# teofum/rust_raytracer

Hardware: AMD Instinct MI355X
Metric: Msamples/sec (whole node), cornell_dragon 870k tri @1000spp (higher is better)
Workload: dtype f64; 1 GPU; scenes/cornell_dragon 1200x1200 @1000spp (10 replicas x 10x10 strata), 871200-tri stand-in mesh; spp=1000, seed=1, pipeline=auto, frames_in_flight=1, partition=1200-row bands round-robin over 1 GPU(s)

## Files before the change

include/rt_mi355.h:

```cpp
#ifndef RT_MI355_H
#define RT_MI355_H

#include <stdint.h>
#include <stddef.h>

#ifdef __cplusplus
extern "C" {
#endif

#define RT_MI355_ABI_VERSION 2

typedef enum RtStatus {
    RT_OK = 0,
    RT_E_INVALID = -1,
    RT_E_UNSUPPORTED = -2,
    RT_E_DEVICE = -3,
    RT_E_NOMEM = -4
} RtStatus;

typedef enum RtNodeType {
    RT_NODE_SPHERE = 1,
    RT_NODE_PLANE = 2,
    RT_NODE_MESH = 3,
    RT_NODE_LIST = 4,
// ... 175 lines not shown
                     const RtRenderParams* params, double* d_rgba_out, void* stream);

int rt_get_stats(const RtScene* scene, RtRenderStats* out);

int rt_debug_trace_sample(const RtScene* scene, const RtCameraDesc* camera, const RtRenderParams* params,
                          uint32_t tid, uint32_t x, uint32_t y, uint32_t sx, uint32_t sy,
                          double* rgb_out, double* trace_out, uint32_t max_bounces);

int rt_debug_fuzzy_reflection(int device, uint32_t n, const double* reflected, const double* fuzz, const uint64_t* state, double* out, uint64_t* state_out);

#define RT_SCENE_INFO_ZERO_WEIGHT_STOP 1u
#define RT_SCENE_INFO_TEX_INTERPRETER 2u
#define RT_SCENE_INFO_VOLUMES 4u
int rt_scene_info(const RtSceneDesc* desc, uint32_t* flags_out);
int rt_scene_mesh_stats(const RtSceneDesc* desc, uint64_t out[8]);
int rt_scene_program(const RtSceneDesc* desc, int32_t* ops_out, uint32_t capacity, uint32_t* n_ops_out, uint64_t info[8]);

int rt_scene_set_tail_flag(RtScene* scene, int32_t* flag);

typedef struct RtAccum RtAccum;
int rt_accum_create(const RtScene* scene, const RtCameraDesc* camera, const RtRenderParams* params, RtAccum** out);
void rt_accum_destroy(RtAccum* acc);
int rt_accum_render(RtAccum* acc, uint32_t n_replicas, const RtRenderParams* params_or_null, void* stream);
uint32_t rt_accum_replicas_done(const RtAccum* acc);
int rt_accum_estimate(const RtAccum* acc, double* rgba_out);
int rt_accum_estimate_device(const RtAccum* acc, double* d_rgba_out, void* stream);
int rt_accum_preview_rgb8(const RtAccum* acc, uint8_t* rgb_out);
size_t rt_accum_state_size(const RtAccum* acc);
int rt_accum_save_state(const RtAccum* acc, void* buf, size_t size);
int rt_accum_load_state(RtAccum* acc, const void* buf, size_t size);
// ... 48 lines not shown
```

rust_raytracer_amd/api.py:

```python
from __future__ import annotations

import ctypes as C
import os
import sys
from typing import Optional, Sequence

import numpy as np

PKG_DIR = os.path.dirname(os.path.abspath(__file__))
REPO_DIR = os.path.dirname(PKG_DIR)

RT_OK = 0
RT_E_INVALID, RT_E_UNSUPPORTED, RT_E_DEVICE, RT_E_NOMEM = -1, -2, -3, -4
RT_PRECISION_F64, RT_PRECISION_F32 = 0, 1
RT_PIPELINE_AUTO, RT_PIPELINE_MEGAKERNEL, RT_PIPELINE_WAVEFRONT = 0, 1, 2
RT_SCENE_BVH_ON_DEVICE = 1
RT_DENOISE_DEMODULATE = 1
RT_DENOISE_MAX_ITERATIONS = 16
AOV_CHANNELS = 8

(RT_NODE_SPHERE, RT_NODE_PLANE, RT_NODE_MESH, RT_NODE_LIST, RT_NODE_TRANSFORM, RT_NODE_BVH,
 RT_NODE_SKY, RT_NODE_SUN, RT_NODE_VOLUME, RT_NODE_NULL) = range(1, 11)
(RT_MAT_LAMBERTIAN, RT_MAT_METAL, RT_MAT_DIELECTRIC, RT_MAT_GLOSSY, RT_MAT_EMISSIVE,
 RT_MAT_ISOTROPIC, RT_MAT_NORMAL_DEBUG) = range(1, 8)
(RT_TEX_CONST_COLOR, RT_TEX_CONST_FLOAT, RT_TEX_CHECKER, RT_TEX_CHECKER_SOLID, RT_TEX_LERP,
 RT_TEX_IMAGE, RT_TEX_NOISE_SOLID, RT_TEX_CHANNEL, RT_TEX_UV_DEBUG) = range(1, 10)


class RtNode(C.Structure):
    _fields_ = [("type", C.c_uint32), ("flags", C.c_uint32), ("material", C.c_int32),
                ("mesh", C.c_int32), ("transform", C.c_int32), ("first_child", C.c_uint32),
# ... 196 lines not shown
        lib.rt_render_device.restype = C.c_int
        lib.rt_get_stats.argtypes = [C.c_void_p, C.POINTER(RtRenderStats)]
        lib.rt_get_stats.restype = C.c_int
        lib.rt_debug_trace_sample.argtypes = [C.c_void_p, C.POINTER(RtCameraDesc), C.POINTER(RtRenderParams),
                                              C.c_uint32, C.c_uint32, C.c_uint32, C.c_uint32, C.c_uint32,
                                              C.POINTER(C.c_double), C.POINTER(C.c_double), C.c_uint32]
        lib.rt_debug_trace_sample.restype = C.c_int
        lib.rt_scene_info.argtypes = [C.POINTER(RtSceneDesc), C.POINTER(C.c_uint32)]
        lib.rt_scene_info.restype = C.c_int
        if hasattr(lib, "rt_scene_set_tail_flag"):
            lib.rt_scene_set_tail_flag.argtypes = [C.c_void_p, C.c_void_p]
            lib.rt_scene_set_tail_flag.restype = C.c_int
        if hasattr(lib, "rt_scene_mesh_stats"):
            lib.rt_scene_mesh_stats.argtypes = [C.POINTER(RtSceneDesc), C.POINTER(C.c_uint64)]
            lib.rt_scene_mesh_stats.restype = C.c_int
        if hasattr(lib, "rt_accum_create"):
            for name, res, args in (
                    ("rt_accum_create", C.c_int, [C.c_void_p, C.POINTER(RtCameraDesc), C.POINTER(RtRenderParams), C.POINTER(C.c_void_p)]),
                    ("rt_accum_destroy", None, [C.c_void_p]),
                    ("rt_accum_render", C.c_int, [C.c_void_p, C.c_uint32, C.POINTER(RtRenderParams), C.c_void_p]),
                    ("rt_accum_replicas_done", C.c_uint32, [C.c_void_p]),
                    ("rt_accum_estimate", C.c_int, [C.c_void_p, C.c_void_p]),
                    ("rt_accum_estimate_device", C.c_int, [C.c_void_p, C.c_void_p, C.c_void_p]),
                    ("rt_accum_preview_rgb8", C.c_int, [C.c_void_p, C.c_void_p]),
                    ("rt_accum_state_size", C.c_size_t, [C.c_void_p]),
                    ("rt_accum_save_state", C.c_int, [C.c_void_p, C.c_void_p, C.c_size_t]),
                    ("rt_accum_load_state", C.c_int, [C.c_void_p, C.c_void_p, C.c_size_t]),
                    ("rt_tonemap_rgb8_device", C.c_int, [C.c_int, C.c_void_p, C.c_uint32, C.c_uint32, C.c_void_p, C.c_void_p])):
                fn = getattr(lib, name)
                fn.argtypes = args
# ... 39 lines not shown
    if st != RT_OK:
        raise RtError(st, lib.rt_last_error().decode())
    return flags.value


def scene_mesh_stats(desc) -> dict:
    lib = load_device_lib()
    out = (C.c_uint64 * 8)()
    st = lib.rt_scene_mesh_stats(desc, out)
    if st != RT_OK:
        raise RtError(st, lib.rt_last_error().decode())
    return dict(zip(("triangles", "bvh2_nodes", "bvh4_nodes", "bvh2_depth", "bvh4_stack", "ops", "rebuilt_groups", "rebuilt_prims"),
                    [int(x) for x in out]))


def scene_program(desc) -> tuple:
    import numpy as np
    lib = load_device_lib()
    lib.rt_scene_program.argtypes = [C.POINTER(RtSceneDesc), C.POINTER(C.c_int32), C.c_uint32, C.POINTER(C.c_uint32), C.POINTER(C.c_uint64)]
    lib.rt_scene_program.restype = C.c_int
    n = C.c_uint32()
    info = (C.c_uint64 * 8)()
    st = lib.rt_scene_program(desc, None, 0, C.byref(n), info)
    if st != RT_OK:
        raise RtError(st, lib.rt_last_error().decode())
    ops = np.zeros((n.value, 4), dtype=np.int32)
    st = lib.rt_scene_program(desc, ops.ctypes.data_as(C.POINTER(C.c_int32)), n.value, C.byref(n), info)
    if st != RT_OK:
        raise RtError(st, lib.rt_last_error().decode())
    plan = int(info[6])
# ... 360 lines not shown
```

rust_raytracer_amd/csrc/rt_bvh.cpp:

```cpp
#include "rt_bvh.h"

#include <algorithm>
#include <cmath>
#include <cstdlib>
#include <limits>

#include "rt_scene.h"

namespace rt {
namespace {

constexpr int kMaxBins = 64;
static int g_bins = 16;
constexpr double kInf = std::numeric_limits<double>::infinity();

struct Box {
    double lo[3] = {kInf, kInf, kInf};
    double hi[3] = {-kInf, -kInf, -kInf};
    void grow(const double* p) {
        for (int a = 0; a < 3; a++) {
            if (p[a] < lo[a]) lo[a] = p[a];
            if (p[a] > hi[a]) hi[a] = p[a];
        }
    }
// ... 214 lines not shown
    c.build(0, 0, 0);
    for (int a = 0; a < 3; a++) { c.out.root_lo[a] = kInf; c.out.root_hi[a] = -kInf; }
    const BuildNodeN<W>& r = c.out.nodes[0];
    for (int k = 0; k < W; k++)
        if (r.child[k] != kEmptyChild)
            for (int a = 0; a < 3; a++) {
                c.out.root_lo[a] = std::min(c.out.root_lo[a], r.lo[k][a]);
                c.out.root_hi[a] = std::max(c.out.root_hi[a], r.hi[k][a]);
            }
    return std::move(c.out);
}
}

Bvh4Build collapse_bvh4(const BvhBuild& b2) { return collapse<4>(b2); }

}
```

rust_raytracer_amd/csrc/rt_bvh.h:

```cpp
#pragma once
#include <cstdint>
#include <string>
#include <vector>

namespace rt {

struct BuildNode {
    double lo0[3], hi0[3], lo1[3], hi1[3];
    int32_t c0, c1;
};

struct BvhBuild {
    std::vector<BuildNode> nodes;
    std::vector<uint32_t> tri_order;
    uint32_t max_depth = 0;
};

BvhBuild build_bvh(const double* positions, const uint32_t* tri_pos, uint32_t n_tris, uint32_t max_leaf);

bool build_bvh_device(const double* positions, uint32_t n_positions, const uint32_t* tri_pos, uint32_t n_tris, uint32_t max_leaf,
                      BvhBuild* out, std::string* err);

template <int W>
struct BuildNodeN {
    double lo[W][3], hi[W][3];
    int32_t child[W];
};
template <int W>
struct BvhNBuild {
    std::vector<BuildNodeN<W>> nodes;
    uint32_t max_depth = 0;
    uint32_t max_stack = 0;
    double root_lo[3], root_hi[3];
};
using BuildNode4 = BuildNodeN<4>;
using Bvh4Build = BvhNBuild<4>;
Bvh4Build collapse_bvh4(const BvhBuild& bvh2);

}
```

rust_raytracer_amd/csrc/rt_kernels.hip:

```cpp
#include <hip/hip_runtime.h>

#include <algorithm>
#include <cmath>
#include <cstdio>
#include <cstdlib>
#include <cstring>
#include <memory>
#include <new>
#include <string>
#include <type_traits>
#include <vector>

#include "rt_aov.h"
#include "rt_compile.h"
#include "rt_device.h"
#include "rt_wavefront.h"

namespace rt {

template <typename R, bool STATS, bool TEX>
__global__ void __launch_bounds__(256) k_megakernel(SceneView<R> sc, CameraView<R> cam, ParamsView<R> prm,
                                                    double* __restrict__ out, DeviceCounters* counters, uint32_t t_first,
                                                    uint32_t n_rep) {
    extern __shared__ int lds_stack[];
// ... 327 lines not shown
            group_nodes.resize(cs.group_nodes4.size());
            for (size_t g = 0; g < cs.groups.size(); g++) {
                const GroupRec<double>& gr = cs.groups[g];
                double S = 0.0;
                for (int a = 0; a < 3; a++) S = std::fmax(S, std::fmax(std::fabs(gr.lo[a]), std::fabs(gr.hi[a])));
                if (!std::isfinite(S)) return set_err(RT_E_UNSUPPORTED, "primitive group with an unbounded box");
                const size_t end = g + 1 < cs.groups.size() ? cs.groups[g + 1].root : cs.group_nodes4.size();
                for (size_t i = gr.root; i < end; i++) {
                    const BuildNode4& sn = cs.group_nodes4[i];
                    BvhNode4q& qn = group_nodes[i];
                    if (!quantise(4, sn.lo, sn.hi, sn.child, S * (1.0 / 524288.0), qn.org, qn.cell, qn.qlo, qn.qhi, qn.child))
                        return set_err(RT_E_UNSUPPORTED, "group BVH node does not fit the 8-bit grid");
                }
            }
        }
        std::vector<Bounds<R>> mesh_bounds(cs.mesh_bounds.size());
        for (size_t i = 0; i < mesh_bounds.size(); i++)
            for (int a = 0; a < 3; a++) {
                mesh_bounds[i].lo[a] = round_down<R>(cs.mesh_bounds[i].lo[a]);
                mesh_bounds[i].hi[a] = round_up<R>(cs.mesh_bounds[i].hi[a]);
            }
        std::vector<TriRec<R>> tris(cs.tris.size());
        for (size_t i = 0; i < tris.size(); i++) {
            cast_arr(tris[i].v0, cs.tris[i].v0); cast_arr(tris[i].e1, cs.tris[i].e1); cast_arr(tris[i].e2, cs.tris[i].e2);
            tris[i]._pad = R(0);
        }
        std::vector<TriAttr<R>> attrs(cs.attrs.size());
        for (size_t i = 0; i < attrs.size(); i++) {
            const auto& s = cs.attrs[i];
            cast_arr(attrs[i].n0, s.n0); cast_arr(attrs[i].n1, s.n1); cast_arr(attrs[i].n2, s.n2);
// ... 28 lines not shown
        std::vector<R> perlin_vec(cs.perlin_vec.size());
        for (size_t i = 0; i < perlin_vec.size(); i++) perlin_vec[i] = R(cs.perlin_vec[i]);
        int st;
        if ((st = buf.upload(cs.ops, &view.ops)) != RT_OK) return st;
        if ((st = buf.upload(bounds, &view.bounds)) != RT_OK) return st;
        if ((st = buf.upload(cs.chain_offsets, &view.chain_offsets)) != RT_OK) return st;
        if ((st = buf.upload(cs.chain_items, &view.chain_items)) != RT_OK) return st;
        if ((st = buf.upload(xforms, &view.xforms)) != RT_OK) return st;
        if ((st = buf.upload(spheres, &view.spheres)) != RT_OK) return st;
        if ((st = buf.upload(planes, &view.planes)) != RT_OK) return st;
        if ((st = buf.upload(suns, &view.suns)) != RT_OK) return st;
        if ((st = buf.upload(cs.meshes, &view.meshes)) != RT_OK) return st;
        if ((st = buf.upload(volumes, &view.volumes)) != RT_OK) return st;
        if ((st = buf.upload(nodes, &view.nodes)) != RT_OK) return st;
        if ((st = buf.upload(nodes4, &view.nodes4)) != RT_OK) return st;
        if ((st = buf.upload(nodes4q, &view.nodes4q)) != RT_OK) return st;
        if ((st = buf.upload(mesh_bounds, &view.mesh_bounds)) != RT_OK) return st;
        if ((st = buf.upload(cs.mesh_ops, &view.mesh_ops)) != RT_OK) return st;
        view.n_mesh_ops = int32_t(cs.mesh_ops.size());
        std::vector<MeshOpRec<R>> mesh_op_recs(cs.mesh_ops.size());
        for (size_t m = 0; m < mesh_op_recs.size(); m++) {
            const Op& op = cs.ops[size_t(cs.mesh_ops[m])];
            const MeshInst& mi = cs.meshes[size_t(op.arg)];
            MeshOpRec<R>& r = mesh_op_recs[m];
            r.pc = cs.mesh_ops[m];
            r.chain = op.chain;
            r.node4_base = mi.node4_base;
            const int32_t cb = cs.chain_offsets[size_t(op.chain)], ce = cs.chain_offsets[size_t(op.chain) + 1];
            r.flags = (mi.flags & 0xFFFFu) | (uint32_t(std::min(ce - cb, 0xFFFF)) << 16);
            for (int a = 0; a < 3; a++) { r.lo[a] = mesh_bounds[size_t(op.arg)].lo[a]; r.hi[a] = mesh_bounds[size_t(op.arg)].hi[a]; }
            for (int k = 0; k < 12; k++) r.inv[k] = ce - cb == 1 ? xforms[size_t(cs.chain_items[size_t(cb)])].inv[k] : R(0);
// ... 346 lines not shown
    if (lds > 160 * 1024) return set_err(RT_E_UNSUPPORTED, "mesh BVH too deep for the LDS traversal stack");
    int n_cu = 0, blocks_per_cu = 0;
    HIP_TRY(hipDeviceGetAttribute(&n_cu, hipDeviceAttributeMultiprocessorCount, s->device));
    const bool stats = p.collect_stats != 0;
    const bool vol = !s->compiled.volumes.empty();
    if (vol) HIP_TRY(hipOccupancyMaxActiveBlocksPerMultiprocessor(&blocks_per_cu, k_wf_intersect<R, false, true>, 256, lds));
    else HIP_TRY(hipOccupancyMaxActiveBlocksPerMultiprocessor(&blocks_per_cu, k_wf_intersect<R, false, false>, 256, lds));
    if (blocks_per_cu < 1) blocks_per_cu = 1;
    const WavefrontPlan plan = plan_wavefront(s->compiled);
    const int n_mesh_ops = int(s->compiled.mesh_ops.size());
    const bool use_split = env_u32("RT_WF_SPLIT", 1) != 0 && plan.split;
    const bool prims_only = use_split && n_mesh_ops == 0;
    const bool split = use_split && n_mesh_ops > 0;
    const bool multi_mesh = plan.multi_mesh || env_u32("RT_WF_MESH_MULTI", 0) != 0;
    const int node_kind = env_u32("RT_WF_NODES", 1) != 0 ? 1 : 0;
    const int mesh_levels = int(s->compiled.max_bvh4_stack) + 1;
    const int lds_levels = std::min<int>(mesh_levels, int(env_u32("RT_WF_LDS_LEVELS", 12)));
    const size_t lds_mesh = size_t(lds_levels) * 256 * sizeof(uint2) + 4 * kMeshWaveLds<R>;
    if (split) {
#define RT_MESH_OCC(ST, ND) do { if (multi_mesh) HIP_TRY(hipOccupancyMaxActiveBlocksPerMultiprocessor(&blocks_per_cu, k_wf_mesh<R, ST, ND, true>, 256, lds_mesh)); \
                                 else HIP_TRY(hipOccupancyMaxActiveBlocksPerMultiprocessor(&blocks_per_cu, k_wf_mesh<R, ST, ND, false>, 256, lds_mesh)); } while (0)
        if (stats) { if (node_kind == 1) RT_MESH_OCC(true, 1); else RT_MESH_OCC(true, 0); }
        else { if (node_kind == 1) RT_MESH_OCC(false, 1); else RT_MESH_OCC(false, 0); }
#undef RT_MESH_OCC
        if (blocks_per_cu < 1) blocks_per_cu = 1;
        blocks_per_cu = std::min<int>(blocks_per_cu, int(env_u32("RT_WF_MESH_BLOCKS", 64)));
    }
    const uint32_t isect_blocks = uint32_t(n_cu) * uint32_t(blocks_per_cu);
    if (split) {
        size_t need = size_t(std::max(mesh_levels - lds_levels, 1)) * isect_blocks * 256 * sizeof(uint2);
// ... 72 lines not shown
        init.cursor = 0;
        init.n_mesh = 0;
        init.next_sample = first;
        *w.h_ctr = init;
        HIP_TRY(hipMemcpyAsync(w.d_ctr, w.h_ctr, sizeof(WfCounters), hipMemcpyHostToDevice, stream));
        if (sparse) hipLaunchKernelGGL((k_wf_generate<R, WfGroupSparse<R>>), dim3((first + 255) / 256), dim3(256), 0, stream, pool, first, grp_s, cv, pv, w.queue[0]);
        else hipLaunchKernelGGL((k_wf_generate<R>), dim3((first + 255) / 256), dim3(256), 0, stream, pool, first, grp, cv, pv, w.queue[0]);
        int qi = 0;
        uint32_t upper = first;
#define RT_LAUNCH_PRIMS(ST, L, VL, GR) hipLaunchKernelGGL((k_wf_prims<R, ST, L, VL, GR>), dim3((upper + WF_CHUNK - 1) / WF_CHUNK), dim3(256), (L ? size_t(staged_prims) : size_t(0)) + (GR ? lds_groups : size_t(0)) + (WF_CHUNK + 4) * 4, stream, ds.view, pool, w.queue[qi], w.mesh_queue, w.d_ctr, s->d_counters, staged_prims, group_levels)
#define RT_LAUNCH_PRIMS_ANY() do { if (vol) { if (stats) RT_LAUNCH_PRIMS(true, 0, true, false); else RT_LAUNCH_PRIMS(false, 0, true, false); } \
                                   else if (groups) { if (stats) { if (lds_prims == 2) RT_LAUNCH_PRIMS(true, 2, false, true); else if (lds_prims == 1) RT_LAUNCH_PRIMS(true, 1, false, true); else RT_LAUNCH_PRIMS(true, 0, false, true); } \
                                                      else { if (lds_prims == 2) RT_LAUNCH_PRIMS(false, 2, false, true); else if (lds_prims == 1) RT_LAUNCH_PRIMS(false, 1, false, true); else RT_LAUNCH_PRIMS(false, 0, false, true); } } \
                                   else if (stats) { if (lds_prims == 1) RT_LAUNCH_PRIMS(true, 1, false, false); else if (lds_prims == 2) RT_LAUNCH_PRIMS(true, 2, false, false); else RT_LAUNCH_PRIMS(true, 0, false, false); } \
                                   else { if (lds_prims == 1) RT_LAUNCH_PRIMS(false, 1, false, false); else if (lds_prims == 2) RT_LAUNCH_PRIMS(false, 2, false, false); else RT_LAUNCH_PRIMS(false, 0, false, false); } } while (0)
#define RT_LAUNCH_MESH_M(ST, ND, MU, QUEUE, NPTR, CPTR) hipLaunchKernelGGL((k_wf_mesh<R, ST, ND, MU>), dim3(isect_blocks), dim3(256), lds_mesh, stream, ds.view, pool, QUEUE, w.d_ctr, s->d_counters, refill_min, inner_min, static_cast<uint2*>(w.mesh_spill), lds_levels, NPTR, CPTR)
#define RT_LAUNCH_MESH_V(ST, ND, QUEUE, NPTR, CPTR) do { if (multi_mesh) RT_LAUNCH_MESH_M(ST, ND, true, QUEUE, NPTR, CPTR); else RT_LAUNCH_MESH_M(ST, ND, false, QUEUE, NPTR, CPTR); } while (0)
#define RT_LAUNCH_MESH(QUEUE, NPTR, CPTR)                                                                                                         \
    do {                                                                                                                                          \
        if (stats) { if (node_kind == 1) RT_LAUNCH_MESH_V(true, 1, QUEUE, NPTR, CPTR); else RT_LAUNCH_MESH_V(true, 0, QUEUE, NPTR, CPTR); } \
        else { if (node_kind == 1) RT_LAUNCH_MESH_V(false, 1, QUEUE, NPTR, CPTR); else RT_LAUNCH_MESH_V(false, 0, QUEUE, NPTR, CPTR); }       \
    } while (0)
        for (;;) {
            size_t ev = 0;
            const bool near_end = s->tail_flag && t0 + nrep >= t_end && w.h_ctr->next_sample + 4ull * pool.capacity >= grp.total;
            const bool all_started = w.h_ctr->next_sample >= grp.total;
            const bool closing = compact_tail && w.h_ctr->next_sample + 2ull * pool.capacity >= grp.total;
            const uint32_t check_now = (compact_tail && all_started) ? 1u : ((near_end || closing) ? std::min<uint32_t>(check_every, 2u) : check_every);
            for (uint32_t k = 0; k < check_now; k++) {
                HIP_TRY(hipEventRecord(w.events[ev++], stream));
                if (split || prims_only) {
// ... 560 lines not shown
    CompileOptions opt;
    if (const char* e = std::getenv("RT_PRIM_REBUILD")) opt.rebuild_prim_groups = std::atoi(e) != 0;
    int st = compile_scene(desc, &cs, &err, opt);
    if (st != RT_OK) return set_err(st, err);
    out[0] = cs.tris.size();
    out[1] = cs.nodes.size();
    out[2] = cs.nodes4.size();
    out[3] = cs.max_bvh_depth;
    out[4] = cs.max_bvh4_stack;
    out[5] = cs.ops.size();
    out[6] = cs.n_rebuilt_groups;
    out[7] = cs.n_rebuilt_prims;
    return RT_OK;
}

int rt_scene_program(const RtSceneDesc* desc, int32_t* ops_out, uint32_t capacity, uint32_t* n_ops_out, uint64_t info[8]) {
    using namespace rt;
    if (!desc || !n_ops_out || !info) return set_err(RT_E_INVALID, "rt_scene_program: NULL argument");
    CompiledScene cs;
    std::string err;
    CompileOptions opt;
    if (const char* e = std::getenv("RT_PRIM_REBUILD")) opt.rebuild_prim_groups = std::atoi(e) != 0;
    int st = compile_scene(desc, &cs, &err, opt);
    if (st != RT_OK) return set_err(st, err);
    *n_ops_out = uint32_t(cs.ops.size());
    if (ops_out)
        for (size_t i = 0; i < cs.ops.size() && i < capacity; i++) {
            ops_out[4 * i + 0] = cs.ops[i].type; ops_out[4 * i + 1] = cs.ops[i].arg;
            ops_out[4 * i + 2] = cs.ops[i].skip; ops_out[4 * i + 3] = cs.ops[i].chain;
        }
// ... 571 lines not shown
```

rust_raytracer_amd/csrc/rt_scene.h:

```cpp
#pragma once
#include <cstdint>

namespace rt {

enum OpType : int32_t {
    OP_END = 0,
    OP_BOUNDS = 1,
    OP_XFORM_PUSH = 2,
    OP_XFORM_POP = 3,
    OP_SPHERE = 4,
    OP_PLANE = 5,
    OP_MESH = 6,
    OP_SKY = 7,
    OP_SUN = 8,
    OP_VOL_BEGIN = 9,
    OP_VOL_MID = 10,
    OP_VOL_END = 11,
    OP_GROUP = 12,
};

struct Op {
    int32_t type;
    int32_t arg;
    int32_t skip;
// ... 87 lines not shown
struct alignas(128) BvhNode4f {
    float lox[4], loy[4], loz[4], hix[4], hiy[4], hiz[4];
    int32_t child[4];
    uint32_t _pad[4];
};

struct alignas(64) BvhNode4q {
    float org[3];
    float cell[3];
    uint32_t qlo[3];
    uint32_t qhi[3];
    int32_t child[4];
};
static_assert(sizeof(BvhNode4q) == 64, "BvhNode4q must be 64 bytes");

template <typename R>
struct alignas(16) TriRec {
    R v0[3], e1[3], e2[3];
    R _pad;
};
template <typename R>
struct alignas(16) TriAttr {
    R n0[3], n1[3], n2[3];
    R uv0[2], uv1[2], uv2[2];
    int32_t has_uv;
    int32_t _pad;
};

struct MaterialRec {
    int32_t type;
// ... 45 lines not shown

template <typename R>
struct SceneView {
    const Op* ops;
    const Bounds<R>* bounds;
    const int32_t* chain_offsets;
    const int32_t* chain_items;
    const Xform<R>* xforms;
    const SpherePrim<R>* spheres;
    const PlanePrim<R>* planes;
    const SunPrim<R>* suns;
    const MeshInst* meshes;
    const VolumeRec<R>* volumes;
    const BvhNode<R>* nodes;
    const BvhNode4f* nodes4;
    const BvhNode4q* nodes4q;
    const Bounds<R>* mesh_bounds;
    const int32_t* mesh_ops;
    const MeshOpRec<R>* mesh_op_recs;
    int32_t n_mesh_ops;
    const GroupRec<R>* groups;
    const BvhNode4q* group_nodes;
    const GroupPrimRef* group_prims;
    const int32_t* group_guards;
    int32_t n_group_nodes;
    int32_t group_stack_levels;
    const TriRec<R>* tris;
    const TriAttr<R>* attrs;
    const MaterialRec* materials;
    const MaterialParams<R>* material_params;
    const TextureRec<R>* textures;
// ... 44 lines not shown
```

rust_raytracer_amd/csrc/rt_wavefront.h:

```cpp
#pragma once
#include "rt_device.h"

#ifndef RT_ISECT_WAVES
#define RT_ISECT_WAVES 3
#endif
#ifndef RT_MESH_WAVES
#define RT_MESH_WAVES 4
#endif
namespace rt {

template <typename R>
struct WfPool {
    uint32_t capacity;
    R *ox, *oy, *oz, *dx, *dy, *dz;
    R *tr, *tg, *tb;
    uint64_t* rng;
    uint64_t* sample;
    uint32_t* depth;
    R *ht, *hu, *hv;
    int32_t *hpc, *htri;
};

template <typename T> RT_DEV T& at(T* base, uint32_t slot) {
    return *reinterpret_cast<T*>(reinterpret_cast<char*>(base) + slot * uint32_t(sizeof(T)));
// ... 627 lines not shown
        if (sp < lds_levels) lds[sp * 256] = (static_cast<unsigned long long>(__float_as_uint(dist)) << 32) | uint32_t(child);
        else spill[size_t(sp - lds_levels) * spill_stride] = make_uint2(uint32_t(child), __float_as_uint(dist));
    }
    RT_DEV uint2 get(int sp) const {
        if (sp < lds_levels) {
            unsigned long long e = lds[sp * 256];
            return make_uint2(uint32_t(e), uint32_t(e >> 32));
        }
        return spill[size_t(sp - lds_levels) * spill_stride];
    }
};

template <typename R> constexpr uint32_t kMeshWaveLds = 1024u + 3u * 64u * uint32_t(sizeof(R));

template <typename R, bool STATS, int NODE, bool MULTI>
__global__ void __launch_bounds__(256, RT_MESH_WAVES) k_wf_mesh(SceneView<R> sc, WfPool<R> pool, const uint32_t* __restrict__ mesh_queue,
                                                                 WfCounters* __restrict__ ctr, DeviceCounters* counters,
                                                                 uint32_t refill_min, uint32_t inner_min,
                                                                 uint2* __restrict__ spill, int lds_levels,
                                                                 const uint32_t* __restrict__ n_ptr, uint32_t* __restrict__ cursor_ptr) {
    extern __shared__ uint2 lds_stack2[];
    MeshStack stk;
    stk.lds = (LdsU64*)(lds_stack2 + threadIdx.x);
    const uint32_t lane = threadIdx.x & 63u;
    char* wave_area = reinterpret_cast<char*>(lds_stack2 + size_t(lds_levels) * 256) + (threadIdx.x >> 6) * kMeshWaveLds<R>;
    uint16_t* pair_tbl = reinterpret_cast<uint16_t*>(wave_area);
    R* res_t = reinterpret_cast<R*>(wave_area + 1024);
    R* res_u = res_t + 64;
    R* res_v = res_u + 64;
    stk.spill = spill + (size_t(blockIdx.x) * blockDim.x + threadIdx.x);
    stk.lds_levels = lds_levels;
    stk.spill_stride = gridDim.x * blockDim.x;
    const uint32_t n = *n_ptr;
    const R t_lo = R(0.001);
    const BvhNode4f* nodes = sc.nodes4;
    const BvhNode4q* nodesq = sc.nodes4q;
    const TriRec<R>* tris = sc.tris;
    const uint32_t n_mesh_ops = uint32_t(sc.n_mesh_ops);
    const R big = sizeof(R) == 8 ? R(1e150) : R(1e18);
    const MeshOpRec<R>* mrecs = sc.mesh_op_recs;
    auto load_rec = [&](uint32_t m, MeshOpRec<R>& rb) {
        const auto* rec = as_const_mem(mrecs) + m;
        rb.pc = rec->pc; rb.chain = rec->chain; rb.node4_base = rec->node4_base; rb.flags = rec->flags;
#pragma unroll
        for (int a = 0; a < 3; a++) { rb.lo[a] = rec->lo[a]; rb.hi[a] = rec->hi[a]; }
#pragma unroll
        for (int k = 0; k < 12; k++) rb.inv[k] = rec->inv[k];
    };
    MeshOpRec<R> rb0;
    if constexpr (!MULTI) load_rec(0u, rb0);
    LaneCounters cnt;
    uint32_t w_node = 0, w_tri = 0, w_refill = 0, l_refill = 0, l_culled = 0;
    bool has = false;
    bool pending = false;
    bool exhausted = false;
    WaveRange range;
    uint32_t slot = 0;
    uint32_t mcur = 0;
    V3<R> o{}, d{};
    R t_max = R(0), hit_u = R(0), hit_v = R(0), t_shift = R(0);
    int32_t hit_tri = -1;
    float ivx = 0.f, ivy = 0.f, ivz = 0.f, oix = 0.f, oiy = 0.f, oiz = 0.f, tmax32 = 0.f;
    int32_t node = 0;
    int sp = 0;

    auto finish_path = [&]() {
        if constexpr (MULTI) {
            const uint32_t hm = (mcur >> 15) & 0x7FFFu;
            if (hm != 0u) {
                at(pool.ht, slot) = t_max; at(pool.hu, slot) = hit_u; at(pool.hv, slot) = hit_v;
                at(pool.hpc, slot) = sc.mesh_ops[hm - 1u]; at(pool.htri, slot) = hit_tri;
            }
        } else {
            if (hit_tri >= 0) {
                at(pool.ht, slot) = t_max; at(pool.hu, slot) = hit_u; at(pool.hv, slot) = hit_v;
                at(pool.hpc, slot) = rb0.pc; at(pool.htri, slot) = hit_tri;
            }
        }
    };
// ... 60 lines not shown
            const R eps = Lim<R>::eps() * R(16);
            if ((t_shift - fabs(t_shift) * eps > t_exit + fabs(t_exit) * eps) || (t_shift - fabs(t_shift) * eps > t_max) || !(rb.lo[0] <= rb.hi[0])) return false;
        }
        if (!(t_shift < Lim<R>::inf())) t_shift = R(0);
        V3<R> oc = o + d * t_shift;
        const float big32 = 1e18f;
        float dx32 = float(d.x), dy32 = float(d.y), dz32 = float(d.z);
        ivx = 1.0f / dx32; ivy = 1.0f / dy32; ivz = 1.0f / dz32;
        ivx = fabsf(ivx) > big32 ? copysignf(big32, ivx) : ivx;
        ivy = fabsf(ivy) > big32 ? copysignf(big32, ivy) : ivy;
        ivz = fabsf(ivz) > big32 ? copysignf(big32, ivz) : ivz;
        oix = float(oc.x) * ivx; oiy = float(oc.y) * ivy; oiz = float(oc.z) * ivz;
        tmax32 = f32_at_least(t_max - t_shift);
        node = int32_t(rb.node4_base);
        sp = 0;
        return true;
    };

    for (;;) {
        if constexpr (MULTI) {
            const unsigned long long idle = __ballot(!has);
            const unsigned long long waiting = __ballot(pending);
            if ((uint32_t(__popcll(idle)) >= refill_min && (!exhausted || waiting != 0ull)) || (waiting != 0ull && idle == ~0ull)) {
                const unsigned long long want = __ballot(!has && !pending);
                if (!exhausted && want != 0ull) {
                    uint32_t my = 0;
                    if (STATS) w_refill++;
                    if (wave_fetch(range, want, cursor_ptr, n, exhausted, my)) {
                        if (STATS) l_refill++;
                        slot = mesh_queue[my];
// ... 46 lines not shown
        }
        for (;;) {
            unsigned long long inner = __ballot(has && node >= 0);
            if (inner == 0ull) break;
            if (uint32_t(__popcll(inner)) < inner_min && __ballot(has && node < 0) != 0ull) break;
            if (STATS) w_node++;
            if (has && node >= 0) {
                if (STATS) cnt.node_visits++;
                const float miss = __builtin_huge_valf();
                float nr[4];
                int32_t ch[4];
                if constexpr (NODE == 1) {
                    const uint4* nd = reinterpret_cast<const uint4*>(nodesq + node);
                    const uint4 h0 = nd[0], h1 = nd[1], h2 = nd[2];
                    const int4 cc = *reinterpret_cast<const int4*>(nd + 3);
                    ch[0] = cc.x; ch[1] = cc.y; ch[2] = cc.z; ch[3] = cc.w;
                    const float ax = __uint_as_float(h0.w) * ivx, ay = __uint_as_float(h1.x) * ivy, az = __uint_as_float(h1.y) * ivz;
                    const float bx = fmaf(__uint_as_float(h0.x), ivx, -oix), by = fmaf(__uint_as_float(h0.y), ivy, -oiy), bz = fmaf(__uint_as_float(h0.z), ivz, -oiz);
                    const bool negx = ivx < 0.0f, negy = ivy < 0.0f, negz = ivz < 0.0f;
                    const uint32_t qnx = negx ? h2.y : h1.z, qfx = negx ? h1.z : h2.y;
                    const uint32_t qny = negy ? h2.z : h1.w, qfy = negy ? h1.w : h2.z;
                    const uint32_t qnz = negz ? h2.w : h2.x, qfz = negz ? h2.x : h2.w;
#pragma unroll
                    for (int k = 0; k < 4; k++) {
                        const float nxk = float((qnx >> (8 * k)) & 0xFFu), nyk = float((qny >> (8 * k)) & 0xFFu), nzk = float((qnz >> (8 * k)) & 0xFFu);
                        const float fxk = float((qfx >> (8 * k)) & 0xFFu), fyk = float((qfy >> (8 * k)) & 0xFFu), fzk = float((qfz >> (8 * k)) & 0xFFu);
                        float tn = fmaxf(fmaxf(fmaf(nxk, ax, bx), fmaf(nyk, ay, by)), fmaxf(fmaf(nzk, az, bz), 0.0f));
                        float tf = fminf(fminf(fmaf(fxk, ax, bx), fmaf(fyk, ay, by)), fminf(fmaf(fzk, az, bz), tmax32));
                        bool h = (tn <= tf) && ch[k] != kEmptyChild;
                        nr[k] = h ? tn : miss;
                    }
// ... 489 lines not shown
```

Measured before the change: 1326 Msamples/s.

## Add normal-cone backface culling to quantized BVH4 mesh traversal

Builds a per-child normal cone (quantized int8 axis plus width) for each quantized BVH4 node and stores it next to the node, padding each node to a 128-byte line. During traversal the ray direction is quantized to int8, and a packed dot product (sdot4) culls children whose triangles all face away from the ray, for meshes that do not hit back faces. This skips node visits and triangle tests on back-facing subtrees, at the cost of doubling the node footprint and extra memory traffic per visit. For the f32 non-stats path it also changes launch bounds to allow five waves.

```diff
diff --git a/include/rt_mi355.h b/include/rt_mi355.h
--- a/include/rt_mi355.h
+++ b/include/rt_mi355.h
@@ -213,6 +213,8 @@
 #define RT_SCENE_INFO_VOLUMES 4u
 int rt_scene_info(const RtSceneDesc* desc, uint32_t* flags_out);
 int rt_scene_mesh_stats(const RtSceneDesc* desc, uint64_t out[8]);
+int rt_scene_mesh_cones(const RtSceneDesc* desc, uint32_t mesh, uint32_t f32, int32_t* children_out, uint32_t* cones_out,
+                        uint32_t node_capacity, uint32_t* n_nodes_out, double* tris_out, uint32_t tri_capacity, uint32_t* n_tris_out);
 int rt_scene_program(const RtSceneDesc* desc, int32_t* ops_out, uint32_t capacity, uint32_t* n_ops_out, uint64_t info[8]);
 
 int rt_scene_set_tail_flag(RtScene* scene, int32_t* flag);
diff --git a/rust_raytracer_amd/api.py b/rust_raytracer_amd/api.py
--- a/rust_raytracer_amd/api.py
+++ b/rust_raytracer_amd/api.py
@@ -15,6 +15,7 @@
 RT_PRECISION_F64, RT_PRECISION_F32 = 0, 1
 RT_PIPELINE_AUTO, RT_PIPELINE_MEGAKERNEL, RT_PIPELINE_WAVEFRONT = 0, 1, 2
 RT_SCENE_BVH_ON_DEVICE = 1
+RT_MESH_HIT_BACK_FACES = 2
 RT_DENOISE_DEMODULATE = 1
 RT_DENOISE_MAX_ITERATIONS = 16
 AOV_CHANNELS = 8
@@ -241,6 +242,10 @@
         if hasattr(lib, "rt_scene_mesh_stats"):
             lib.rt_scene_mesh_stats.argtypes = [C.POINTER(RtSceneDesc), C.POINTER(C.c_uint64)]
             lib.rt_scene_mesh_stats.restype = C.c_int
+        if hasattr(lib, "rt_scene_mesh_cones"):
+            lib.rt_scene_mesh_cones.argtypes = [C.POINTER(RtSceneDesc), C.c_uint32, C.c_uint32, C.c_void_p, C.c_void_p, C.c_uint32,
+                                                C.POINTER(C.c_uint32), C.c_void_p, C.c_uint32, C.POINTER(C.c_uint32)]
+            lib.rt_scene_mesh_cones.restype = C.c_int
         if hasattr(lib, "rt_accum_create"):
             for name, res, args in (
                     ("rt_accum_create", C.c_int, [C.c_void_p, C.POINTER(RtCameraDesc), C.POINTER(RtRenderParams), C.POINTER(C.c_void_p)]),
@@ -310,6 +315,23 @@
                     [int(x) for x in out]))
 
 
+def scene_mesh_cones(desc, mesh: int = 0, f32: bool = False) -> tuple:
+    import numpy as np
+    lib = load_device_lib()
+    nn, nt = C.c_uint32(), C.c_uint32()
+    st = lib.rt_scene_mesh_cones(desc, mesh, int(f32), None, None, 0, C.byref(nn), None, 0, C.byref(nt))
+    if st != RT_OK:
+        raise RtError(st, lib.rt_last_error().decode())
+    children = np.zeros((nn.value, 4), dtype=np.int32)
+    cones = np.zeros((nn.value, 4), dtype=np.uint32)
+    tris = np.zeros((nt.value, 3, 3), dtype=np.float64)
+    st = lib.rt_scene_mesh_cones(desc, mesh, int(f32), children.ctypes.data, cones.ctypes.data, nn.value, C.byref(nn),
+                                 tris.ctypes.data, nt.value, C.byref(nt))
+    if st != RT_OK:
+        raise RtError(st, lib.rt_last_error().decode())
+    return children, cones.view(np.int8).reshape(-1, 4, 4), tris
+
+
 def scene_program(desc) -> tuple:
     import numpy as np
     lib = load_device_lib()
diff --git a/rust_raytracer_amd/csrc/rt_bvh.cpp b/rust_raytracer_amd/csrc/rt_bvh.cpp
--- a/rust_raytracer_amd/csrc/rt_bvh.cpp
+++ b/rust_raytracer_amd/csrc/rt_bvh.cpp
@@ -252,4 +252,108 @@
 
 Bvh4Build collapse_bvh4(const BvhBuild& b2) { return collapse<4>(b2); }
 
-}
+
+namespace {
+constexpr double kConeDirSlack = 0.00682;
+constexpr double kConeSafety = 0.001;
+constexpr double kConeMinCos = 0.125;
+}
+
+ConeLimits cone_limits(bool f32) {
+    if (f32) return ConeLimits{1.0 / 32.0, 1e-12, 1e12};
+    return ConeLimits{1.0 / 1048576.0, 1e-100, 1e100};
+}
+
+void build_mesh_cones(const std::vector<BuildNode4>& nodes4, const std::vector<TriRec<double>>& tris, const ConeLimits& lim,
+                      std::vector<uint32_t>* out) {
+    const size_t n_tris = tris.size();
+    std::vector<double> normal(3 * n_tris);
+    const double kNaN = std::numeric_limits<double>::quiet_NaN();
+    for (size_t t = 0; t < n_tris; t++) {
+        const TriRec<double>& r = tris[t];
+        const double* a = r.e1;
+        const double* b = r.e2;
+        const double cx = a[1] * b[2] - a[2] * b[1], cy = a[2] * b[0] - a[0] * b[2], cz = a[0] * b[1] - a[1] * b[0];
+        const double la = std::sqrt(a[0] * a[0] + a[1] * a[1] + a[2] * a[2]), lb = std::sqrt(b[0] * b[0] + b[1] * b[1] + b[2] * b[2]);
+        const double lc = std::sqrt(cx * cx + cy * cy + cz * cz);
+        bool ok = std::isfinite(r.v0[0]) && std::isfinite(r.v0[1]) && std::isfinite(r.v0[2]);
+        ok = ok && la >= lim.min_edge && la <= lim.max_edge && lb >= lim.min_edge && lb <= lim.max_edge;
+        ok = ok && lc >= lim.sigma * la * lb && lc > 0.0;
+        normal[3 * t] = ok ? cx / lc : kNaN;
+        normal[3 * t + 1] = ok ? cy / lc : kNaN;
+        normal[3 * t + 2] = ok ? cz / lc : kNaN;
+    }
+    struct Below {
+        uint32_t lo = UINT32_MAX, hi = 0, count = 0;
+        double sum[3] = {0.0, 0.0, 0.0};
+        void add(const Below& o) {
+            lo = std::min(lo, o.lo); hi = std::max(hi, o.hi); count += o.count;
+            for (int a = 0; a < 3; a++) sum[a] += o.sum[a];
+        }
+    };
+    auto cone_around = [&](const Below& b, const double* axis) -> uint32_t {
+        const double l = std::sqrt(axis[0] * axis[0] + axis[1] * axis[1] + axis[2] * axis[2]);
+        if (!(l > 0.0) || !std::isfinite(l)) return kNeutralCone;
+        int q[3];
+        double al = 0.0;
+        for (int a = 0; a < 3; a++) { q[a] = int(std::lround(127.0 * axis[a] / l)); al += double(q[a]) * double(q[a]); }
+        al = std::sqrt(al);
+        if (!(al > 0.0)) return kNeutralCone;
+        const double ax = q[0] / al, ay = q[1] / al, az = q[2] / al;
+        double c = 1.0;
+        for (uint32_t t = b.lo; t < b.hi; t++) {
+            c = std::min(c, ax * normal[3 * size_t(t)] + ay * normal[3 * size_t(t) + 1] + az * normal[3 * size_t(t) + 2]);
+            if (c < kConeMinCos) return kNeutralCone;
+        }
+        if (!(c >= kConeMinCos)) return kNeutralCone;
+        const double s = std::sqrt(std::max(0.0, 1.0 - c * c));
+        const double w = std::ceil(al * (s + kConeDirSlack + kConeSafety));
+        if (!(w >= 1.0 && w <= 127.0)) return kNeutralCone;
+        return uint32_t(q[0] & 0xFF) | (uint32_t(q[1] & 0xFF) << 8) | (uint32_t(q[2] & 0xFF) << 16) | (uint32_t(w) << 24);
+    };
+    auto cone_word = [&](const Below& b) -> uint32_t {
+        if (b.count == 0 || b.hi - b.lo != b.count) return kNeutralCone;
+        uint32_t word = cone_around(b, b.sum);
+        if (word == kNeutralCone && b.count >= 2 && b.count <= 8 && std::isfinite(b.sum[0])) {
+            uint32_t bi = b.lo, bj = b.lo;
+            double least = 2.0;
+            for (uint32_t i = b.lo; i < b.hi; i++)
+                for (uint32_t j = i + 1; j < b.hi; j++) {
+                    const double* ni = &normal[3 * size_t(i)];
+                    const double* nj = &normal[3 * size_t(j)];
+                    const double dij = ni[0] * nj[0] + ni[1] * nj[1] + ni[2] * nj[2];
+                    if (dij < least) { least = dij; bi = i; bj = j; }
+                }
+            const double mid[3] = {normal[3 * size_t(bi)] + normal[3 * size_t(bj)], normal[3 * size_t(bi) + 1] + normal[3 * size_t(bj) + 1],
+                                   normal[3 * size_t(bi) + 2] + normal[3 * size_t(bj) + 2]};
+            word = cone_around(b, mid);
+        }
+        return word;
+    };
+    out->assign(4 * nodes4.size(), kNeutralCone);
+    std::vector<Below> below(nodes4.size());
+    for (size_t i = nodes4.size(); i-- > 0;) {
+        const BuildNode4& nd = nodes4[i];
+        Below all;
+        for (int k = 0; k < 4; k++) {
+            const int32_t ch = nd.child[k];
+            if (ch == kEmptyChild) continue;
+            Below b;
+            if (ch >= 0) {
+                if (size_t(ch) <= i || size_t(ch) >= nodes4.size()) { all.sum[0] = kNaN; continue; }
+                b = below[size_t(ch)];
+            } else {
+                const uint32_t code = uint32_t(~ch), first = code >> 3, count = (code & 7u) + 1u;
+                if (size_t(first) + count > n_tris) { all.sum[0] = kNaN; continue; }
+                b.lo = first; b.hi = first + count; b.count = count;
+                for (uint32_t t = first; t < first + count; t++)
+                    for (int a = 0; a < 3; a++) b.sum[a] += normal[3 * size_t(t) + a];
+            }
+            (*out)[4 * i + size_t(k)] = cone_word(b);
+            all.add(b);
+        }
+        below[i] = all;
+    }
+}
+
+}
diff --git a/rust_raytracer_amd/csrc/rt_bvh.h b/rust_raytracer_amd/csrc/rt_bvh.h
--- a/rust_raytracer_amd/csrc/rt_bvh.h
+++ b/rust_raytracer_amd/csrc/rt_bvh.h
@@ -2,6 +2,8 @@
 #include <cstdint>
 #include <string>
 #include <vector>
+
+#include "rt_scene.h"
 
 namespace rt {
 
@@ -37,4 +39,13 @@
 using Bvh4Build = BvhNBuild<4>;
 Bvh4Build collapse_bvh4(const BvhBuild& bvh2);
 
+struct ConeLimits {
+    double sigma;
+    double min_edge;
+    double max_edge;
+};
+ConeLimits cone_limits(bool f32);
+void build_mesh_cones(const std::vector<BuildNode4>& nodes4, const std::vector<TriRec<double>>& tris, const ConeLimits& lim,
+                      std::vector<uint32_t>* out);
+
 }
diff --git a/rust_raytracer_amd/csrc/rt_kernels.hip b/rust_raytracer_amd/csrc/rt_kernels.hip
--- a/rust_raytracer_amd/csrc/rt_kernels.hip
+++ b/rust_raytracer_amd/csrc/rt_kernels.hip
@@ -365,6 +365,14 @@
                 }
             }
         }
+        std::vector<uint32_t> cone_words;
+        build_mesh_cones(cs.nodes4, cs.tris, cone_limits(sizeof(R) == 4), &cone_words);
+        std::vector<MeshNode4qc> nodes4qc(cs.nodes4.size());
+        for (size_t i = 0; i < nodes4qc.size(); i++) {
+            nodes4qc[i].node = nodes4q[i];
+            for (int k = 0; k < 4; k++) nodes4qc[i].cones.word[k] = cone_words[4 * i + size_t(k)];
+            for (uint32_t& x : nodes4qc[i]._pad) x = 0;
+        }
         std::vector<Bounds<R>> mesh_bounds(cs.mesh_bounds.size());
         for (size_t i = 0; i < mesh_bounds.size(); i++)
             for (int a = 0; a < 3; a++) {
@@ -423,7 +431,7 @@
         if ((st = buf.upload(volumes, &view.volumes)) != RT_OK) return st;
         if ((st = buf.upload(nodes, &view.nodes)) != RT_OK) return st;
         if ((st = buf.upload(nodes4, &view.nodes4)) != RT_OK) return st;
-        if ((st = buf.upload(nodes4q, &view.nodes4q)) != RT_OK) return st;
+        if ((st = buf.upload(nodes4qc, &view.nodes4q)) != RT_OK) return st;
         if ((st = buf.upload(mesh_bounds, &view.mesh_bounds)) != RT_OK) return st;
         if ((st = buf.upload(cs.mesh_ops, &view.mesh_ops)) != RT_OK) return st;
         view.n_mesh_ops = int32_t(cs.mesh_ops.size());
@@ -800,6 +808,7 @@
     const bool split = use_split && n_mesh_ops > 0;
     const bool multi_mesh = plan.multi_mesh || env_u32("RT_WF_MESH_MULTI", 0) != 0;
     const int node_kind = env_u32("RT_WF_NODES", 1) != 0 ? 1 : 0;
+    const uint32_t cones_on = env_u32("RT_WF_CONES", 1) != 0 ? 1u : 0u;
     const int mesh_levels = int(s->compiled.max_bvh4_stack) + 1;
     const int lds_levels = std::min<int>(mesh_levels, int(env_u32("RT_WF_LDS_LEVELS", 12)));
     const size_t lds_mesh = size_t(lds_levels) * 256 * sizeof(uint2) + 4 * kMeshWaveLds<R>;
@@ -902,7 +911,7 @@
                                                       else { if (lds_prims == 2) RT_LAUNCH_PRIMS(false, 2, false, true); else if (lds_prims == 1) RT_LAUNCH_PRIMS(false, 1, false, true); else RT_LAUNCH_PRIMS(false, 0, false, true); } } \
                                    else if (stats) { if (lds_prims == 1) RT_LAUNCH_PRIMS(true, 1, false, false); else if (lds_prims == 2) RT_LAUNCH_PRIMS(true, 2, false, false); else RT_LAUNCH_PRIMS(true, 0, false, false); } \
                                    else { if (lds_prims == 1) RT_LAUNCH_PRIMS(false, 1, false, false); else if (lds_prims == 2) RT_LAUNCH_PRIMS(false, 2, false, false); else RT_LAUNCH_PRIMS(false, 0, false, false); } } while (0)
-#define RT_LAUNCH_MESH_M(ST, ND, MU, QUEUE, NPTR, CPTR) hipLaunchKernelGGL((k_wf_mesh<R, ST, ND, MU>), dim3(isect_blocks), dim3(256), lds_mesh, stream, ds.view, pool, QUEUE, w.d_ctr, s->d_counters, refill_min, inner_min, static_cast<uint2*>(w.mesh_spill), lds_levels, NPTR, CPTR)
+#define RT_LAUNCH_MESH_M(ST, ND, MU, QUEUE, NPTR, CPTR) hipLaunchKernelGGL((k_wf_mesh<R, ST, ND, MU>), dim3(isect_blocks), dim3(256), lds_mesh, stream, ds.view, pool, QUEUE, w.d_ctr, s->d_counters, refill_min, inner_min, static_cast<uint2*>(w.mesh_spill), lds_levels, NPTR, CPTR, cones_on)
 #define RT_LAUNCH_MESH_V(ST, ND, QUEUE, NPTR, CPTR) do { if (multi_mesh) RT_LAUNCH_MESH_M(ST, ND, true, QUEUE, NPTR, CPTR); else RT_LAUNCH_MESH_M(ST, ND, false, QUEUE, NPTR, CPTR); } while (0)
 #define RT_LAUNCH_MESH(QUEUE, NPTR, CPTR)                                                                                                         \
     do {                                                                                                                                          \
@@ -1493,6 +1502,47 @@
     return RT_OK;
 }
 
+int rt_scene_mesh_cones(const RtSceneDesc* desc, uint32_t mesh, uint32_t f32, int32_t* children_out, uint32_t* cones_out,
+                        uint32_t node_capacity, uint32_t* n_nodes_out, double* tris_out, uint32_t tri_capacity, uint32_t* n_tris_out) {
+    using namespace rt;
+    if (!desc || !n_nodes_out || !n_tris_out) return set_err(RT_E_INVALID, "rt_scene_mesh_cones: NULL argument");
+    CompiledScene cs;
+    std::string err;
+    int st = compile_scene(desc, &cs, &err, CompileOptions());
+    if (st != RT_OK) return set_err(st, err);
+    if (mesh >= cs.meshes.size()) return set_err(RT_E_INVALID, "rt_scene_mesh_cones: mesh index out of range");
+    const MeshInst& mi = cs.meshes[mesh];
+    size_t node_end = cs.nodes4.size();
+    for (const MeshInst& o : cs.meshes)
+        if (o.node4_base > mi.node4_base) node_end = std::min(node_end, size_t(o.node4_base));
+    const size_t n_nodes = node_end - mi.node4_base;
+    *n_nodes_out = uint32_t(n_nodes);
+    *n_tris_out = mi.n_tris;
+    if (children_out && cones_out) {
+        std::vector<uint32_t> words;
+        build_mesh_cones(cs.nodes4, cs.tris, cone_limits(f32 != 0), &words);
+        for (size_t i = 0; i < n_nodes && i < node_capacity; i++)
+            for (int k = 0; k < 4; k++) {
+                int32_t ch = cs.nodes4[mi.node4_base + i].child[k];
+                if (ch != kEmptyChild) {
+                    if (ch >= 0) ch -= int32_t(mi.node4_base);
+                    else {
+                        const uint32_t code = uint32_t(~ch);
+                        ch = ~int32_t((((code >> 3) - mi.tri_base) << 3) | (code & 7u));
+                    }
+                }
+                children_out[4 * i + size_t(k)] = ch;
+                cones_out[4 * i + size_t(k)] = words[4 * (mi.node4_base + i) + size_t(k)];
+            }
+    }
+    if (tris_out)
+        for (size_t t = 0; t < mi.n_tris && t < tri_capacity; t++) {
+            const TriRec<double>& r = cs.tris[mi.tri_base + t];
+            for (int a = 0; a < 3; a++) { tris_out[9 * t + size_t(a)] = r.v0[a]; tris_out[9 * t + 3 + size_t(a)] = r.e1[a]; tris_out[9 * t + 6 + size_t(a)] = r.e2[a]; }
+        }
+    return RT_OK;
+}
+
 int rt_scene_program(const RtSceneDesc* desc, int32_t* ops_out, uint32_t capacity, uint32_t* n_ops_out, uint64_t info[8]) {
     using namespace rt;
     if (!desc || !n_ops_out || !info) return set_err(RT_E_INVALID, "rt_scene_program: NULL argument");
diff --git a/rust_raytracer_amd/csrc/rt_scene.h b/rust_raytracer_amd/csrc/rt_scene.h
--- a/rust_raytracer_amd/csrc/rt_scene.h
+++ b/rust_raytracer_amd/csrc/rt_scene.h
@@ -125,6 +125,18 @@
 };
 static_assert(sizeof(BvhNode4q) == 64, "BvhNode4q must be 64 bytes");
 
+struct alignas(16) NodeCones4 {
+    uint32_t word[4];
+};
+struct alignas(128) MeshNode4qc {
+    BvhNode4q node;
+    NodeCones4 cones;
+    uint32_t _pad[12];
+};
+static_assert(sizeof(MeshNode4qc) == 128, "one cache line per mesh node");
+constexpr uint32_t kNeutralCone = 0x7F000000u;
+constexpr uint32_t kNoCullDir = 0x81000000u;
+
 template <typename R>
 struct alignas(16) TriRec {
     R v0[3], e1[3], e2[3];
@@ -200,7 +212,7 @@
     const VolumeRec<R>* volumes;
     const BvhNode<R>* nodes;
     const BvhNode4f* nodes4;
-    const BvhNode4q* nodes4q;
+    const MeshNode4qc* nodes4q;
     const Bounds<R>* mesh_bounds;
     const int32_t* mesh_ops;
     const MeshOpRec<R>* mesh_op_recs;
diff --git a/rust_raytracer_amd/csrc/rt_wavefront.h b/rust_raytracer_amd/csrc/rt_wavefront.h
--- a/rust_raytracer_amd/csrc/rt_wavefront.h
+++ b/rust_raytracer_amd/csrc/rt_wavefront.h
@@ -665,11 +665,12 @@
 template <typename R> constexpr uint32_t kMeshWaveLds = 1024u + 3u * 64u * uint32_t(sizeof(R));
 
 template <typename R, bool STATS, int NODE, bool MULTI>
-__global__ void __launch_bounds__(256, RT_MESH_WAVES) k_wf_mesh(SceneView<R> sc, WfPool<R> pool, const uint32_t* __restrict__ mesh_queue,
+__global__ void __launch_bounds__(256, (sizeof(R) == 4 && !STATS && NODE == 1) ? 5 : RT_MESH_WAVES) k_wf_mesh(SceneView<R> sc, WfPool<R> pool, const uint32_t* __restrict__ mesh_queue,
                                                                  WfCounters* __restrict__ ctr, DeviceCounters* counters,
                                                                  uint32_t refill_min, uint32_t inner_min,
                                                                  uint2* __restrict__ spill, int lds_levels,
-                                                                 const uint32_t* __restrict__ n_ptr, uint32_t* __restrict__ cursor_ptr) {
+                                                                 const uint32_t* __restrict__ n_ptr, uint32_t* __restrict__ cursor_ptr,
+                                                                 uint32_t cones_on) {
     extern __shared__ uint2 lds_stack2[];
     MeshStack stk;
     stk.lds = (LdsU64*)(lds_stack2 + threadIdx.x);
@@ -685,7 +686,7 @@
     const uint32_t n = *n_ptr;
     const R t_lo = R(0.001);
     const BvhNode4f* nodes = sc.nodes4;
-    const BvhNode4q* nodesq = sc.nodes4q;
+    const MeshNode4qc* nodesq = sc.nodes4q;
     const TriRec<R>* tris = sc.tris;
     const uint32_t n_mesh_ops = uint32_t(sc.n_mesh_ops);
     const R big = sizeof(R) == 8 ? R(1e150) : R(1e18);
@@ -714,6 +715,7 @@
     float ivx = 0.f, ivy = 0.f, ivz = 0.f, oix = 0.f, oiy = 0.f, oiz = 0.f, tmax32 = 0.f;
     int32_t node = 0;
     int sp = 0;
+    uint32_t dirq = kNoCullDir;
 
     auto finish_path = [&]() {
         if constexpr (MULTI) {
@@ -804,6 +806,16 @@
         tmax32 = f32_at_least(t_max - t_shift);
         node = int32_t(rb.node4_base);
         sp = 0;
+        if constexpr (NODE == 1) {
+            const R len2 = d.x * d.x + d.y * d.y + d.z * d.z;
+            const R len_lo = sizeof(R) == 8 ? R(1e-200) : R(1e-24), len_hi = sizeof(R) == 8 ? R(1e200) : R(1e24);
+            dirq = kNoCullDir;
+            if (cones_on != 0u && (rb.flags & RT_MESH_HIT_BACK_FACES) == 0u && len2 > len_lo && len2 < len_hi) {
+                const R sc127 = R(127) / sqrt(len2);
+                const int qx = int(rint(d.x * sc127)), qy = int(rint(d.y * sc127)), qz = int(rint(d.z * sc127));
+                dirq = (uint32_t(qx) & 0xFFu) | ((uint32_t(qy) & 0xFFu) << 8) | ((uint32_t(qz) & 0xFFu) << 16) | kNoCullDir;
+            }
+        }
         return true;
     };
 
@@ -880,7 +892,11 @@
                     const uint4* nd = reinterpret_cast<const uint4*>(nodesq + node);
                     const uint4 h0 = nd[0], h1 = nd[1], h2 = nd[2];
                     const int4 cc = *reinterpret_cast<const int4*>(nd + 3);
-                    ch[0] = cc.x; ch[1] = cc.y; ch[2] = cc.z; ch[3] = cc.w;
+                    const uint4 cn = nd[4];
+                    ch[0] = __builtin_amdgcn_sdot4(int(dirq), int(cn.x), 0, false) > 0 ? kEmptyChild : cc.x;
+                    ch[1] = __builtin_amdgcn_sdot4(int(dirq), int(cn.y), 0, false) > 0 ? kEmptyChild : cc.y;
+                    ch[2] = __builtin_amdgcn_sdot4(int(dirq), int(cn.z), 0, false) > 0 ? kEmptyChild : cc.z;
+                    ch[3] = __builtin_amdgcn_sdot4(int(dirq), int(cn.w), 0, false) > 0 ? kEmptyChild : cc.w;
                     const float ax = __uint_as_float(h0.w) * ivx, ay = __uint_as_float(h1.x) * ivy, az = __uint_as_float(h1.y) * ivz;
                     const float bx = fmaf(__uint_as_float(h0.x), ivx, -oix), by = fmaf(__uint_as_float(h0.y), ivy, -oiy), bz = fmaf(__uint_as_float(h0.z), ivz, -oiz);
                     const bool negx = ivx < 0.0f, negy = ivy < 0.0f, negz = ivz < 0.0f;
```

After: 1424 Msamples/s, median of 6. 1.07x the previous value.
